# bruniss/multi-task-3d-resencoder-unet

Measured on AMD Instinct MI355X. Metric: train patches/sec (b,c,z,y,x) ResEncM 1x128^3, higher is better.
Workload: dtype bf16; 1 GPU; cfg2: ResEncM (6 stages, feats [32, 64, 128, 256, 512, 512], blocks [1, 3, 4, 6, 6, 6]), 1-in, heads ['sheet'], patch 128x128x128, batch 2/GPU, full train step (fwd+loss+bwd+allreduce+clip+AdamW); global_batch=2, parallelism=dp1

## Files before the change

include/rxunet.h:

```cpp
#ifndef RXUNET_H
#define RXUNET_H

#include <stddef.h>
#include <stdint.h>

#ifdef __cplusplus
extern "C" {
#endif

#define RX_OK 0
#define RX_EINVAL (-1)
#define RX_EUNSUPPORTED (-2)
#define RX_ELAUNCH (-3)
#define RX_EWORKSPACE (-4)

typedef enum { RX_F32 = 0, RX_BF16 = 1, RX_F16 = 2 } rx_dtype;
typedef enum { RX_ACT_NONE = 0, RX_ACT_SIGMOID = 1, RX_ACT_SOFTMAX = 2 } rx_head_act;

typedef struct {
  void* ptr;
  int32_t n, z, y, x, c, ld;
  int64_t cs;
} rx_act;

int rx_abi_version(void);
const char* rx_last_error(void);
int rx_device_arch_ok(void);
const char* rx_last_conv_kernel(void);

int rx_pack_conv_weight(rx_dtype dt, const float* w, int co, int ci, int taps, void* w_fwd, void* w_bwd,
                        void* stream);
int rx_pack_convT_weight(rx_dtype dt, const float* w, int ci, int co, int taps, void* w_fwd, void* w_bwd,
                         void* stream);
int rx_pack_multi(rx_dtype dt, int count, const float* const* w, const int* kind, const int* A, const int* B,
                  const int* taps, void* const* w_fwd, void* const* w_bwd, void* stream);

size_t rx_conv_workspace_hint(void);
int rx_conv3d_fwd(rx_dtype dt, const rx_act* x, const void* w_fwd, const float* bias, const rx_act* y,
                  const int32_t kernel[3], const int32_t stride[3], void* ws, size_t ws_bytes, void* stream);
int rx_conv3d_fwd_stats(rx_dtype dt, const rx_act* x, const void* w_fwd, const float* bias, const rx_act* y,
                        const int32_t kernel[3], const int32_t stride[3], float eps, float* stats, void* ws,
                        size_t ws_bytes, void* stream);
int rx_conv3d_bwd_data(rx_dtype dt, const rx_act* dy, const void* w_bwd, const rx_act* dx,
                       const int32_t kernel[3], const int32_t stride[3], int accumulate, void* ws,
                       size_t ws_bytes, void* stream);
int rx_conv3d_bwd_data_instats(rx_dtype dt, const rx_act* dy, const void* w_bwd, const rx_act* dx,
                               const int32_t kernel[3], const int32_t stride[3], int accumulate, const rx_act* in_y,
                               const float* in_stats, float slope, float* m12, int* fused, void* ws, size_t ws_bytes,
                               void* stream);
size_t rx_conv3d_bwd_weight_workspace(const rx_act* x, const rx_act* dy, const int32_t kernel[3]);
int rx_conv3d_bwd_weight(rx_dtype dt, const rx_act* x, const rx_act* dy, float* dw, const int32_t kernel[3],
                         const int32_t stride[3], void* ws, size_t ws_bytes, void* stream);

int rx_convT3d_fwd(rx_dtype dt, const rx_act* x, const void* w_fwd, const float* bias, const rx_act* y,
                   const int32_t stride[3], void* ws, size_t ws_bytes, void* stream);
int rx_convT3d_bwd_data(rx_dtype dt, const rx_act* dy, const void* w_bwd, const rx_act* dx,
                        const int32_t stride[3], int accumulate, void* ws, size_t ws_bytes, void* stream);
size_t rx_convT3d_bwd_weight_workspace(const rx_act* x, const rx_act* dy, const int32_t stride[3]);
int rx_convT3d_bwd_weight(rx_dtype dt, const rx_act* x, const rx_act* dy, float* dw, const int32_t stride[3],
                          void* ws, size_t ws_bytes, void* stream);

size_t rx_instnorm_stats_workspace(const rx_act* y);
int rx_instnorm_stats(rx_dtype dt, const rx_act* y, float eps, float* stats, void* ws, size_t ws_bytes,
                      void* stream);
int rx_instnorm_stats_mask(float* stats, const float* keep, int count, void* stream);
int rx_instnorm_act_fwd(rx_dtype dt, const rx_act* y, const float* stats, const rx_act* residual,
                        const rx_act* out, float slope, void* stream);
int rx_instnorm_fwd(rx_dtype dt, const rx_act* y, float eps, float* stats, const rx_act* residual,
                    const rx_act* out, float slope, void* ws, size_t ws_bytes, void* stream);
int rx_instnorm_act_bwd(rx_dtype dt, const rx_act* g, const rx_act* y, const float* stats, const rx_act* out,
                        float slope, const rx_act* dy, const rx_act* d_residual, int accumulate_residual,
                        void* ws, size_t ws_bytes, void* stream);

int rx_instnorm_act_bwd_res(rx_dtype dt, const rx_act* g, const rx_act* y, const float* stats, const rx_act* out,
                            float slope, const rx_act* pool_dy, const int32_t pool_stride[3], const rx_act* d_residual,
                            const rx_act* dy, void* ws, size_t ws_bytes, void* stream);

int rx_instnorm_act_bwd_apply(rx_dtype dt, const rx_act* g, const rx_act* y, const float* stats, const rx_act* out,
                              float slope, const float* m12, const rx_act* dy, const rx_act* d_residual,
                              int accumulate_residual, void* stream);

typedef struct {
  const float* w1;
  const float* b1;
  const float* w2;
// ... 144 lines not shown
```

multi-task-3d-resencoder-unet_amd/csrc/rx_wgrad_halo.hip:

```cpp
#include <stdlib.h>

#include <type_traits>

#include "rx_common.h"

struct WgHaloGeom {
  int N, Z, Y, X;
  int R, Cc, ldg, ldx;
  long g_ss, x_ss;
  long x_cs;
  int TZ, TY, TX, lTX, lTY;
  int HY, HX, HV, VT;
  int tz_n, ty_n, tx_n, NT;
  int S, tiles_per_split, panels_c;
  int sz, sy, sx;
  int Zi, Yi, Xi;
  int order;
  int dbg;
};

typedef __attribute__((address_space(3))) s16x4 lds_s16x4_h;

#define RX_WGH_MAX_HV 768
#define RX_WGH_MAX_VT 256
#define RX_WGH_XPIECES ((RX_WGH_MAX_HV * 4 + 255) / 256)
#define RX_WGH_GPIECES (RX_WGH_MAX_VT * 4 / 256)

template <typename T>
__device__ inline u32x4 tr_frag(const T* p0, const T* p1) {
  s16x4 t0 = __builtin_amdgcn_ds_read_tr16_b64_v4i16((lds_s16x4_h*)(p0));
  s16x4 t1 = __builtin_amdgcn_ds_read_tr16_b64_v4i16((lds_s16x4_h*)(p1));
  u32x2 lo = __builtin_bit_cast(u32x2, t0), hi = __builtin_bit_cast(u32x2, t1);
  return u32x4{lo[0], lo[1], hi[0], hi[1]};
}

template <typename T>
__global__ __launch_bounds__(256, 2) void wgrad_halo_kernel(const T* __restrict__ gt, const T* __restrict__ xt, float* __restrict__ slab,
                                                            float* __restrict__ dw, const WgHaloGeom g) {
  extern __shared__ __attribute__((aligned(16))) unsigned char smem[];
  T* sG = reinterpret_cast<T*>(smem);
  T* sX = sG + RX_WGH_MAX_VT * 32;

  const int tid = threadIdx.x, lane = tid & 63;
  const int wave = __builtin_amdgcn_readfirstlane(tid >> 6);
  const int PPn = gridDim.x, lid = rx_xcd_remap(blockIdx.y * PPn + blockIdx.x, PPn * gridDim.y);
  const int split = lid / PPn, pp = lid - split * PPn;
  const int pr = pp / g.panels_c, pc = pp - pr * g.panels_c;
  const int r0 = pr * 32, c0 = pc * 32;
  const long xc0 = g.x_cs ? (long)pc * g.x_cs : (long)c0;
  const int t_begin = split * g.tiles_per_split;
  const int t_end = min(g.NT, t_begin + g.tiles_per_split);

  const int chunk = tid & 3;
  int xh[RX_WGH_XPIECES];
#pragma unroll
  for (int p = 0; p < RX_WGH_XPIECES; ++p) {
    int row = (tid >> 2) + 64 * p;
    if (row < g.HV) {
      int hx = row % g.HX, t = row / g.HX;
      int hy = t % g.HY, hz = t / g.HY;
      xh[p] = (hz << 16) | (hy << 8) | hx;
    } else
      xh[p] = -1;
  }

  const int g16 = lane >> 4, half = g16 & 1, h = g16 >> 1, l15 = lane & 15, q4 = l15 >> 2, p4 = l15 & 3;
  const int coloff = 16 * half + 4 * p4;
  int toff[7];
#pragma unroll
  for (int j = 0; j < 7; ++j) {
    int t = wave + 4 * j;
    int dz = t / 9 - 1, dy = (t / 3) % 3 - 1, dx = t % 3 - 1;
    toff[j] = t < 27 ? ((dz * g.HY + dy) * g.HX + dx) * 32 : 0;
  }

  f32x16 acc[7];
#pragma unroll
  for (int j = 0; j < 7; ++j)
#pragma unroll
// ... 43 lines not shown
      int row = (tid >> 2) + 64 * p;
      if (xh[p] >= 0) *reinterpret_cast<u32x4*>(sX + row * 32 + chunk * 8) = xv[p];
    }
    __syncthreads();
    if (tile + 1 < t_end) load_tile(tile + 1);
    for (int s = 0; s < ksteps; ++s) {
      const int v = 16 * s + 8 * h + q4;
      const int vx = v & (g.TX - 1), vy = (v >> g.lTX) & (g.TY - 1), vz = v >> (g.lTX + g.lTY);
      const int hr = ((vz * g.sz + 1) * g.HY + (vy * g.sy + 1)) * g.HX + vx * g.sx + 1;
      int hr4;
      if (g.TX >= 8)
        hr4 = hr + 4 * g.sx;
      else {
        const int v2 = v + 4;
        const int vy2 = (v2 >> g.lTX) & (g.TY - 1), vz2 = v2 >> (g.lTX + g.lTY);
        hr4 = ((vz2 * g.sz + 1) * g.HY + (vy2 * g.sy + 1)) * g.HX + (v2 & (g.TX - 1)) * g.sx + 1;
      }
      const u32x4 a = tr_frag<T>(sG + v * 32 + coloff, sG + (v + 4) * 32 + coloff);
      const T* b0 = sX + hr * 32 + coloff;
      const T* b1 = sX + hr4 * 32 + coloff;
      u32x4 bf[7];
#pragma unroll
      for (int j = 0; j < 7; ++j)
        if (j < 6 || wave < 3) bf[j] = tr_frag<T>(b0 + toff[j], b1 + toff[j]);
      __builtin_amdgcn_sched_barrier(0);
#pragma unroll
      for (int j = 0; j < 7; ++j)
        if (j < 6 || wave < 3) Mma<T>::run(acc[j], a, bf[j]);
      __builtin_amdgcn_sched_barrier(0);
    }
  }

  const int col = lane & 31, fh = lane >> 5;
  if (g.S == 1) {
    float* sT = reinterpret_cast<float*>(smem);
#pragma unroll
    for (int hb = 0; hb < 2; ++hb) {
      __syncthreads();
#pragma unroll
      for (int j = 0; j < 7; ++j) {
        const int t = wave + 4 * j;
        if (t < 27) {
#pragma unroll
          for (int r = 8 * hb; r < 8 * hb + 8; ++r) {
            const int lr = (r & 3) + 8 * ((r >> 2) & 1) + 4 * fh;
            sT[(lr * 32 + col) * 27 + t] = acc[j][r];
          }
        }
      }
      __syncthreads();
      for (int idx = tid; idx < 16 * 216; idx += 256) {
        const int lr = idx / 216, i = idx - lr * 216;
        *reinterpret_cast<f32x4*>(dw + ((long)(r0 + 16 * hb + lr) * g.Cc + c0) * 27 + 4 * i) = *reinterpret_cast<const f32x4*>(sT + 4 * idx);
      }
    }
    return;
  }
#pragma unroll
  for (int j = 0; j < 7; ++j) {
    const int t = wave + 4 * j;
    if (t < 27) {
      float* out = slab + (((long)split * 27 + t) * g.R + r0) * g.Cc + c0;
#pragma unroll
      for (int r = 0; r < 16; ++r) {
        const int row = (r & 3) + 8 * (r >> 2) + 4 * fh;
        out[(long)row * g.Cc + col] = acc[j][r];
      }
    }
  }
}


typedef __attribute__((address_space(3))) unsigned char lds_byte;

__device__ inline u32x4 tr_frag_at(const lds_byte* p, int off0, int off1) {
  s16x4 t0 = __builtin_amdgcn_ds_read_tr16_b64_v4i16((lds_s16x4_h*)(p + off0));
  s16x4 t1 = __builtin_amdgcn_ds_read_tr16_b64_v4i16((lds_s16x4_h*)(p + off1));
  u32x2 lo = __builtin_bit_cast(u32x2, t0), hi = __builtin_bit_cast(u32x2, t1);
  return u32x4{lo[0], lo[1], hi[0], hi[1]};
}

#define WGH16_HY 6
#define WGH16_HX 18
#define WGH16_HV 648
#define WGH16_XPIECES 11

template <typename T, int W, typename Stage>
__device__ __forceinline__ void wgh16_tile_mma(const lds_byte* gb, const lds_byte* xb, f32x16 (&acc)[7], Stage&& stage) {
  constexpr int NT = W < 3 ? 7 : 6;
  u32x4 fa[2], fb[7];
  auto read_a = [&](int s) { return tr_frag_at(gb, s * 1024, s * 1024 + 256); };
  auto read_b = [&](int s, int j) {
    const int vy = s & 3, vz = s >> 2;
    const int t = W + 4 * j;
    const int dz = t / 9, dy = (t / 3) % 3, dx = t % 3;
    const int off = (((vz + dz) * WGH16_HY + (vy + dy)) * WGH16_HX + dx) * 64;
    return tr_frag_at(xb, off, off + 256);
  };
  fa[0] = read_a(0);
#pragma unroll
  for (int j = 0; j < NT; ++j) fb[j] = read_b(0, j);
#pragma unroll
// ... 283 lines not shown
                        ((long)g.N * g.x_ss + (g.x_cs ? (long)(g.Cc / 32 - 1) * g.x_cs : 0)) * 2 < 0x7fffff00L;
    if (dma_ok && dt == RX_BF16)
      hipLaunchKernelGGL((wgrad_halo16ws_kernel<bf16_t, true>), grid, dim3(512), 2 * lds16, st, (const bf16_t*)dy->ptr, (const bf16_t*)x->ptr, (float*)ws, dw, g);
    else if (dma_ok)
      hipLaunchKernelGGL((wgrad_halo16ws_kernel<f16_t, true>), grid, dim3(512), 2 * lds16, st, (const f16_t*)dy->ptr, (const f16_t*)x->ptr, (float*)ws, dw, g);
    else if (dt == RX_BF16)
      hipLaunchKernelGGL((wgrad_halo16ws_kernel<bf16_t, false>), grid, dim3(512), 2 * lds16, st, (const bf16_t*)dy->ptr, (const bf16_t*)x->ptr, (float*)ws, dw, g);
    else
      hipLaunchKernelGGL((wgrad_halo16ws_kernel<f16_t, false>), grid, dim3(512), 2 * lds16, st, (const f16_t*)dy->ptr, (const f16_t*)x->ptr, (float*)ws, dw, g);
    if (g.S > 1) rx_wgrad_reduce_launch((const float*)ws, g.S, 27, g.R, g.Cc, dw, st);
    hipError_t e16 = hipGetLastError();
    if (e16 != hipSuccess) {
      rx_set_error("wgrad_halo16: %s", hipGetErrorString(e16));
      return RX_ELAUNCH;
    }
    return 1;
  }
  rx_note_kernel("wgrad_halo_kernel");
  if (dt == RX_BF16) {
    (void)hipFuncSetAttribute(reinterpret_cast<const void*>(&wgrad_halo_kernel<bf16_t>), hipFuncAttributeMaxDynamicSharedMemorySize, (int)lds);
    hipLaunchKernelGGL((wgrad_halo_kernel<bf16_t>), grid, dim3(256), lds, st, (const bf16_t*)dy->ptr, (const bf16_t*)x->ptr, (float*)ws, dw, g);
  } else {
    (void)hipFuncSetAttribute(reinterpret_cast<const void*>(&wgrad_halo_kernel<f16_t>), hipFuncAttributeMaxDynamicSharedMemorySize, (int)lds);
    hipLaunchKernelGGL((wgrad_halo_kernel<f16_t>), grid, dim3(256), lds, st, (const f16_t*)dy->ptr, (const f16_t*)x->ptr, (float*)ws, dw, g);
  }
  if (g.S > 1) rx_wgrad_reduce_launch((const float*)ws, g.S, 27, g.R, g.Cc, dw, st);
  hipError_t e = hipGetLastError();
  if (e != hipSuccess) {
    rx_set_error("wgrad_halo: %s", hipGetErrorString(e));
    return RX_ELAUNCH;
  }
  return 1;
}
```

multi-task-3d-resencoder-unet_amd/engine/lib.py:

```python
import ctypes
import os
from ctypes import POINTER, c_char_p, c_double, c_float, c_int, c_int32, c_long, c_size_t, c_void_p

import torch

_HERE = os.path.dirname(os.path.abspath(__file__))
LIB_PATH = os.environ.get("RX_LIBRARY") or os.path.join(os.path.dirname(_HERE), "csrc", "librxunet.so")

RX_F32, RX_BF16, RX_F16 = 0, 1, 2
RX_ACT_NONE, RX_ACT_SIGMOID, RX_ACT_SOFTMAX = 0, 1, 2
DTYPE_CODE = {torch.float32: RX_F32, torch.bfloat16: RX_BF16, torch.float16: RX_F16}
RX_SW_U8, RX_SW_U16, RX_SW_F32 = 0, 1, 2
RX_SW_SCALE, RX_SW_ZSCORE = 0, 1
RX_SW_BLEND_AVERAGE, RX_SW_BLEND_UNIT, RX_SW_BLEND_NONE = 0, 1, 2
RX_SW_CAST_U8, RX_SW_CAST_U16 = 0, 1
RX_AUG_PW_NONE, RX_AUG_PW_AFFINE, RX_AUG_PW_PLANE, RX_AUG_PW_NOISE = 0, 1, 2, 3
RX_AUG_G3_NONE, RX_AUG_G3_FILTER, RX_AUG_G3_DOWNSCALE = 0, 1, 2
RX_AUG_MAX_K, RX_AUG_MAX_BOXES = 21, 4


class RxError(RuntimeError):
    pass


class RxAct(ctypes.Structure):
    _fields_ = [("ptr", c_void_p), ("n", c_int32), ("z", c_int32), ("y", c_int32), ("x", c_int32),
                ("c", c_int32), ("ld", c_int32), ("cs", ctypes.c_int64)]


class RxSeParams(ctypes.Structure):
    _fields_ = [("w1", c_void_p), ("b1", c_void_p), ("w2", c_void_p), ("b2", c_void_p), ("rd", c_int32),
                ("keep_x", c_int32)]


I3 = c_int32 * 3
_P = POINTER(RxAct)
_PSE = POINTER(RxSeParams)

_SIGNATURES = {
    "rx_abi_version": (c_int, []),
    "rx_last_error": (c_char_p, []),
    "rx_device_arch_ok": (c_int, []),
    "rx_last_conv_kernel": (c_char_p, []),
    "rx_pack_conv_weight": (c_int, [c_int, c_void_p, c_int, c_int, c_int, c_void_p, c_void_p, c_void_p]),
    "rx_pack_convT_weight": (c_int, [c_int, c_void_p, c_int, c_int, c_int, c_void_p, c_void_p, c_void_p]),
    "rx_pack_multi": (c_int, [c_int, c_int, c_void_p, c_void_p, c_void_p, c_void_p, c_void_p, c_void_p, c_void_p, c_void_p]),
    "rx_conv_workspace_hint": (c_size_t, []),
    "rx_conv3d_fwd": (c_int, [c_int, _P, c_void_p, c_void_p, _P, I3, I3, c_void_p, c_size_t, c_void_p]),
    "rx_conv3d_fwd_stats": (c_int, [c_int, _P, c_void_p, c_void_p, _P, I3, I3, c_float, c_void_p, c_void_p, c_size_t, c_void_p]),
    "rx_conv3d_bwd_data": (c_int, [c_int, _P, c_void_p, _P, I3, I3, c_int, c_void_p, c_size_t, c_void_p]),
    "rx_conv3d_bwd_data_instats": (c_int, [c_int, _P, c_void_p, _P, I3, I3, c_int, _P, c_void_p, c_float, c_void_p, POINTER(c_int),
                                           c_void_p, c_size_t, c_void_p]),
    "rx_instnorm_act_bwd_apply": (c_int, [c_int, _P, _P, c_void_p, _P, c_float, c_void_p, _P, _P, c_int, c_void_p]),
    "rx_conv3d_bwd_weight_workspace": (c_size_t, [_P, _P, I3]),
    "rx_conv3d_bwd_weight": (c_int, [c_int, _P, _P, c_void_p, I3, I3, c_void_p, c_size_t, c_void_p]),
    "rx_convT3d_fwd": (c_int, [c_int, _P, c_void_p, c_void_p, _P, I3, c_void_p, c_size_t, c_void_p]),
    "rx_convT3d_bwd_data": (c_int, [c_int, _P, c_void_p, _P, I3, c_int, c_void_p, c_size_t, c_void_p]),
    "rx_convT3d_bwd_weight_workspace": (c_size_t, [_P, _P, I3]),
    "rx_convT3d_bwd_weight": (c_int, [c_int, _P, _P, c_void_p, I3, c_void_p, c_size_t, c_void_p]),
    "rx_instnorm_stats_workspace": (c_size_t, [_P]),
    "rx_instnorm_stats": (c_int, [c_int, _P, c_float, c_void_p, c_void_p, c_size_t, c_void_p]),
    "rx_instnorm_act_fwd": (c_int, [c_int, _P, c_void_p, _P, _P, c_float, c_void_p]),
    "rx_instnorm_stats_mask": (c_int, [c_void_p, c_void_p, c_int, c_void_p]),
    "rx_instnorm_fwd": (c_int, [c_int, _P, c_float, c_void_p, _P, _P, c_float, c_void_p, c_size_t, c_void_p]),
    "rx_instnorm_act_bwd": (c_int, [c_int, _P, _P, c_void_p, _P, c_float, _P, _P, c_int, c_void_p, c_size_t,
                                    c_void_p]),
    "rx_instnorm_act_bwd_res": (c_int, [c_int, _P, _P, c_void_p, _P, c_float, _P, I3, _P, _P, c_void_p, c_size_t, c_void_p]),
    "rx_se_workspace": (c_size_t, [_P]),
    "rx_se_gate_fwd": (c_int, [c_int, _P, c_void_p, c_void_p, _PSE, c_void_p, c_void_p, c_void_p, c_void_p, c_void_p, c_size_t,
                               c_void_p]),
    "rx_instnorm_gate_act_fwd": (c_int, [c_int, _P, c_void_p, c_void_p, c_int, _P, _P, c_float, c_void_p]),
    "rx_se_gate_bwd": (c_int, [c_int, _P, _P, c_void_p, _P, c_float, c_void_p, _PSE, c_void_p, c_void_p, c_void_p, c_void_p,
                               c_void_p, c_void_p, c_void_p, c_void_p, c_void_p, c_void_p, c_void_p, c_size_t, c_void_p]),
    "rx_instnorm_gate_act_bwd": (c_int, [c_int, _P, _P, c_void_p, _P, c_float, c_void_p, c_void_p, c_void_p, c_int, _P, _P,
                                         c_int, c_void_p]),
    "rx_avgpool_fwd": (c_int, [c_int, _P, _P, I3, c_void_p]),
    "rx_instnorm_act_pool_fwd": (c_int, [c_int, _P, c_void_p, _P, _P, _P, I3, c_float, c_void_p]),
    "rx_avgpool_bwd": (c_int, [c_int, _P, _P, I3, c_int, c_void_p]),
    "rx_stem_conv_fwd": (c_int, [c_int, c_void_p, c_int, c_int, c_int, c_int, c_int, c_void_p, c_void_p, _P, I3,
                                 c_void_p]),
    "rx_stem_conv_fwd_stats": (c_int, [c_int, c_void_p, c_int, c_int, c_int, c_int, c_int, c_void_p, c_void_p, _P, I3,
                                       c_float, c_void_p, c_void_p, c_size_t, c_void_p]),
    "rx_stem_conv_bwd_weight_workspace": (c_size_t, [c_int, c_int, c_int]),
    "rx_stem_conv_bwd_weight": (c_int, [c_int, c_void_p, c_int, c_int, c_int, c_int, c_int, _P, c_void_p, I3,
                                        c_void_p, c_size_t, c_void_p]),
    "rx_head_fwd": (c_int, [c_int, _P, c_void_p, c_void_p, c_int, c_void_p, c_int, c_void_p]),
    "rx_head_bwd_workspace": (c_size_t, [_P, c_int]),
    "rx_instnorm_act_head_fwd": (c_int, [c_int, _P, c_void_p, _P, c_float, c_void_p, c_void_p, c_int, c_void_p, c_int, c_void_p]),
# ... 100 lines not shown
```

multi-task-3d-resencoder-unet_amd/engine/ops.py:

```python
from ctypes import byref, c_void_p

import numpy as np
import torch

from . import lib as _l
from .lib import I3, RxAct, check, load, stream_ptr

_WS = {}
_PROF = None


def set_profiler(p):
    global _PROF
    _PROF = p


class LaunchProfiler:

    def __init__(self):
        self.pending = []
        self.groups = {}
        self.pending_hbm = []
        self.hbm = {}

# ... 302 lines not shown

    def go():
        check(load().rx_conv3d_bwd_data_instats(_code(dy.dtype), byref(dy.desc()), _ptr(w_bwd), byref(dx.desc()), I3(*kernel),
                                                I3(*stride), int(accumulate), byref(in_y.desc()), _ptr(in_stats), float(slope),
                                                _ptr(m12), byref(fused), *_ws_args(ws), stream_ptr()), "rx_conv3d_bwd_data_instats")
    if _PROF is None:
        go()
    else:
        n = dx.dims[0]
        _PROF.run("dgrad:" + LaunchProfiler.igemm_name(dx.voxels, dx.c), 2.0 * n * dx.voxels * dx.c * dy.c * _taps(kernel), 1, go)
    return bool(fused.value)


def instnorm_act_bwd_apply(g, y, stats, out, dy, m12, slope=0.01, d_residual=None, accumulate_residual=False):
    check(load().rx_instnorm_act_bwd_apply(_code(y.dtype), byref(g.desc()), byref(y.desc()), _ptr(stats),
                                           byref(out.desc()) if out is not None else None, float(slope), _ptr(m12),
                                           byref(dy.desc()),
                                           byref(d_residual.desc()) if d_residual is not None else None,
                                           int(accumulate_residual), stream_ptr()), "rx_instnorm_act_bwd_apply")


def conv3d_bwd_weight(x, dy, dw, kernel, stride, ws=None):
    need = load().rx_conv3d_bwd_weight_workspace(byref(x.desc()), byref(dy.desc()), I3(*kernel))
    ws = workspace(need) if ws is None else ws

    def go():
        check(load().rx_conv3d_bwd_weight(_code(x.dtype), byref(x.desc()), byref(dy.desc()), _ptr(dw), I3(*kernel),
                                          I3(*stride), *_ws_args(ws), stream_ptr()), "rx_conv3d_bwd_weight")
    if _PROF is None:
        return go()
    n = dy.dims[0]
    name = f"wgrad:wgrad_kernel<{64 if dy.c % 64 == 0 else 32},{64 if x.c % 64 == 0 else 32}>"
    _PROF.run(name, 2.0 * n * dy.voxels * dy.c * x.c * _taps(kernel), 1, go)


def convT3d_fwd(x, w_fwd, bias, y, stride, ws=None):
    ws = workspace() if ws is None else ws
    check(load().rx_convT3d_fwd(_code(x.dtype), byref(x.desc()), _ptr(w_fwd), _ptr(bias), byref(y.desc()),
                                I3(*stride), *_ws_args(ws), stream_ptr()), "rx_convT3d_fwd")


def convT3d_bwd_data(dy, w_bwd, dx, stride, accumulate=False, ws=None):
    ws = workspace() if ws is None else ws
    check(load().rx_convT3d_bwd_data(_code(dy.dtype), byref(dy.desc()), _ptr(w_bwd), byref(dx.desc()), I3(*stride),
                                     int(accumulate), *_ws_args(ws), stream_ptr()), "rx_convT3d_bwd_data")


def convT3d_bwd_weight(x, dy, dw, stride, ws=None):
    need = load().rx_convT3d_bwd_weight_workspace(byref(x.desc()), byref(dy.desc()), I3(*stride))
    ws = workspace(need) if ws is None else ws
    check(load().rx_convT3d_bwd_weight(_code(x.dtype), byref(x.desc()), byref(dy.desc()), _ptr(dw), I3(*stride),
                                       *_ws_args(ws), stream_ptr()), "rx_convT3d_bwd_weight")


def instnorm_stats(y, stats, eps=1e-5, ws=None):
    ws = workspace() if ws is None else ws
    check(load().rx_instnorm_stats(_code(y.dtype), byref(y.desc()), eps, _ptr(stats), *_ws_args(ws), stream_ptr()),
          "rx_instnorm_stats")


def instnorm_stats_mask(stats, keep):
    check(load().rx_instnorm_stats_mask(_ptr(stats), _ptr(keep), int(keep.numel()), stream_ptr()), "rx_instnorm_stats_mask")


def instnorm_act_fwd(y, stats, out, slope=0.01, residual=None):
    check(load().rx_instnorm_act_fwd(_code(y.dtype), byref(y.desc()), _ptr(stats),
# ... 309 lines not shown
```

multi-task-3d-resencoder-unet_amd/engine/plan.py:

```python
from dataclasses import dataclass, field
from typing import Callable, Dict, List, Optional

import os

import torch
from torch import nn

from . import lib as _l
from . import ops
from .ops import Act


class UnsupportedConfig(NotImplementedError):
    pass


_SIDE_STREAMS: Dict[str, "torch.cuda.Stream"] = {}


def side_stream(device):
    key = str(device)
    st = _SIDE_STREAMS.get(key)
    if st is None:
        st = _SIDE_STREAMS[key] = torch.cuda.Stream(device=device)
# ... 48 lines not shown
            _l.require_device()
        self.net = net
        self.dtype = dtype
        self.device = device
        self.needs_grad = needs_grad
        self.in_shape = tuple(in_shape)
        self.generation = 0
        self.two_d = net.op_dims == 2
        B, Cin = in_shape[0], in_shape[1]
        spatial = tuple(in_shape[2:])
        if self.two_d:
            spatial = (1,) + spatial
        self.B, self.Cin, self.spatial = B, Cin, spatial

        self.params: List[nn.Parameter] = []
        self._pidx: Dict[int, int] = {}
        self.packs: List[dict] = []
        self.enc_tape: List[Rec] = []
        self.dec_tapes: List[List[Rec]] = []
        self.fwd: List[Callable] = []
        self.bwd: List[Callable] = []
        self.dy_pool: Dict[tuple, Act] = {}
        self._gbase: Dict[int, torch.Tensor] = {}
        self.outputs: Dict[str, torch.Tensor] = {}
        self.bytes_alloc = 0
        self._x = None
        self._dlogits: Dict[str, torch.Tensor] = {}
        self._grads: List[Optional[torch.Tensor]] = []
        self.grad_order: List[int] = []
        self.grad_sync = None
        import os
        self.overlap_wgrad = os.environ.get("RX_OVERLAP_WGRAD", "1") != "0"
        self.dy_ring = 4
        self._side = None
        self._ws2 = None
        self._dy_turn: Dict[tuple, int] = {}
        self._dy_free: Dict[int, int] = {}
        self._dy_ev: Dict[int, int] = {}
        self._ev_fork = None
        self._ev_join = None
        self._pack_groups = None
        self._gates: List[dict] = []
        self._drops: List[dict] = []
        self._shadows: List[dict] = []
        self._shadow_of: Dict[int, dict] = {}
        self._pad_idx: Dict[int, dict] = {}
        self._pad_done: List[int] = []
        self.use_programs = os.environ.get("RX_PROGRAMS", "1") == "1"
        self._pstate: Dict[tuple, dict] = {}
        self._gflat = None
        self._gviews: Dict[int, torch.Tensor] = {}
        self._marks: List[tuple] = []
        self._recording = None
        self._on_side = False
        self._use_gstore = False
        self._gflat_range = (0, 0)
        self._pack_slots: List[int] = []
        self._unstable_params = False
        self._ws_refs: List[object] = []
        self._raw_seen = None
        self.use_graphs = os.environ.get("RX_GRAPHS", "0") == "1"
        self._gstate: Dict[tuple, dict] = {}
        self._x_static = None
        self._dl_static: Dict[str, torch.Tensor] = {}
        self._image_t = None
        self._pack_delay_at = None
# ... 491 lines not shown
                            ops.instnorm_act_fwd(a["y"].act, a["stats"], a["out"].act, a["slope"], res)
                        elif a["drop"] is not None and a["drop"]["active"]:
                            ops.instnorm_stats(a["y"].act, a["stats"], P._eps_now(a))
                            P._mask_dropped(a)
                            ops.instnorm_act_fwd(a["y"].act, a["stats"], a["out"].act, a["slope"], res)
                        else:
                            ops.instnorm_fwd(a["y"].act, a["stats"], a["out"].act, a["slope"], res, a["eps"])
                    f.append(step)
                elif rec.kind == "pool":
                    if not a.get("fused"):
                        f.append(lambda a=a: ops.avgpool_fwd(a["x"].act, a["y"].act, a["stride"]))
                elif rec.kind == "copy":
                    f.append(lambda a=a: ops.avgpool_fwd(a["x"].act, a["y"].act, (1, 1, 1)))
                elif rec.kind == "head":
                    if a.get("fwd_fused"):
                        continue

                    def step(a=a):
                        w2 = a["w"].view(a["k"], -1)
                        ops.head_fwd(a["x"].act, w2, a["b"], a["out"], a["act"] if P._apply_act else _l.RX_ACT_NONE)
                    f.append(step)

    def _dy_for(self, y: AT):
        key = (y.act.dims, y.act.c)
        turn = self._dy_turn.get(key, 0)
        self._dy_turn[key] = (turn + 1) % self.dy_ring
        slot = key + (turn,)
        if slot not in self.dy_pool:
            t = torch.empty((*y.act.dims, y.act.c), dtype=self.dtype, device=self.device)
            self.bytes_alloc += t.numel() * t.element_size()
            self.dy_pool[slot] = Act(t)
        return self.dy_pool[slot]

    def _gen_backward(self):
        P = self
        b = self.bwd
        cat_written = {}

        def mark_cat(cat):
            cat_written[cat.act.key] = True

        def view_written(at):
            return at.written or cat_written.get(at.act.key, False)

        def new_grad(idx):
            sync = P.grad_sync
            ent = P._pad_idx.get(idx)
            if ent is not None:
                if ent["gpad"] is None:
                    ent["gpad"] = torch.empty(tuple(ent["sh"].shape), dtype=torch.float32, device=P.device)
                P._pad_done.append(idx)
                return ent["gpad"]
            if sync is not None:
                g = sync.alloc(idx)
            elif P._use_gstore:
                g = P._gviews[idx]
            else:
                g = torch.empty_like(P.params[idx], memory_format=torch.contiguous_format)
            P._grads[idx] = g
            return g

        skip = set(filter(None, os.environ.get("RX_SKIP", "").split(",")))
        if skip and os.environ.get("RX_ABLATION", "0") != "1":
            raise _l.RxError("RX_SKIP drops launches from the backward pass (timing ablations, wrong gradients): "
                             "set RX_ABLATION=1 as well to confirm, or unset RX_SKIP")

# ... 2 lines not shown
                return
            if P._recording is not None:
                P._marks.append((len(P._recording), idx, P._on_side))
            if P.grad_sync is not None:
                P.grad_sync.ready(idx)

        dy_free = self._dy_free

        def side_run(fn, dy_act):
            if not (P.overlap_wgrad and P._side is not None):
                fn(ops.workspace())
                return
            ops.event_record(P._ev_fork)
            ops.stream_wait(P._ev_fork, P._side)
            key = id(dy_act.t)
            slot = P._dy_ev.get(key)
            if slot is None:
                slot = P._dy_ev[key] = ops.event_new()
            P._on_side = True
            try:
                with torch.cuda.stream(P._side):
                    fn(P._ws2)
                    ops.event_record(slot)
            finally:
                P._on_side = False
            dy_free[key] = slot

        def before_dy_write(dy_act):
            slot = dy_free.pop(id(dy_act.t), None)
            if slot is not None:
                ops.stream_wait(slot)

        order = self.grad_order

        def wrote(at, kind, info=None):
            at._gw = (kind, info)

        for tape in self.dec_tapes + [self.enc_tape]:
            for rec in reversed(tape):
                a = rec.a
                if rec.kind == "head":
                    x = a["x"]
                    assert not view_written(x)
                    gx = self._grad_buf(x)
                    x.written = True
                    hinfo = {"fused": False}
                    wrote(x, "head", hinfo)
                    a["hinfo"] = hinfo

                    def step(a=a, gx=gx, hinfo=hinfo):
                        dl = P._dlogits.get(a["name"])
                        if dl is None:
                            gx.t.zero_()
                            if P.grad_sync is not None:
                                for i in (a["widx"], a["bidx"]):
                                    new_grad(i).zero_()
                                    done(i)
                            return
                        if hinfo.get("dw_fused"):
                            return
                        dw, db = new_grad(a["widx"]), new_grad(a["bidx"])
                        ops.head_bwd(dl, a["x"].act, a["w"].view(a["k"], -1), None if hinfo["fused"] else gx, dw, db)
                        done(a["widx"])
                        done(a["bidx"])
                    order += [a["widx"], a["bidx"]]
                    b.append(step)
                elif rec.kind == "inact":
                    out, y, res = a["out"], a["y"], a["res"]
                    gout = self._grad_buf(out) if out.gact is None else out.gact
                    if not view_written(out):
                        raise RuntimeError(f"plan bug: gradient of {out.name} is consumed before it is produced")
                    dy = self._dy_for(y)
                    y.gact = dy
                    gres, acc = None, False
                    if res is not None and res.needs_grad:
                        gres = self._grad_buf(res)
                        acc = view_written(res)
                        res.written = True
                        wrote(res, "gres")
                    gw = getattr(out, "_gw", (None, None))
                    if (gw[0] == "head" and a["gate"] is None and res is None and self.dtype != torch.float32
                            and out.act.voxels > 512):
                        heads = [r.a for r in tape if r.kind == "head" and r.a["x"] is out]
                        if len(heads) == 1 and heads[0]["k"] <= 4:
                            a["head_src"] = heads[0]
                            gw[1]["fused"] = True
                            if heads[0].get("fwd_fused") and heads[0]["w"] is self.params[heads[0]["widx"]]:
                                a["head_dw_fused"] = True
                                gw[1]["dw_fused"] = True
                    if (gw[0] == "conv" and a["gate"] is None and res is None and self.dtype != torch.float32
                            and out.act.full_buffer and out.act.root is None and out.act.c % 32 == 0 and out.act.voxels > 512
                            and out.act.dims[3] >= 16):
                        a["m12"] = torch.empty((self.B, out.act.c, 2), dtype=torch.float32, device=self.device)
                        a["m12_valid"] = False
                        gw[1]["inact"] = a
                    def gistep(a=a, gout=gout, dy=dy, gres=gres, acc=acc):
                        g = a["gate"]
                        before_dy_write(dy)
                        if g["se"] is None and g.get("scale_now") is None:
                            ops.instnorm_act_bwd(gout, a["y"].act, a["stats"],
                                                 a["out"].act if (a["slope"] != 1.0 and a["res"] is not None) else None, dy,
                                                 a["slope"], gres, acc)
                            return
                        grads = [new_grad(i) for i in g["se"]["idx"]] if g["se"] is not None else [None] * 4
                        ops.se_gate_bwd(gout, a["y"].act, a["stats"], a["out"].act, a["slope"], P._se_args(g), g["pooled"],
# ... 22 lines not shown
                            ops.instnorm_act_bwd_res(gout, a["y"].act, a["stats"], a["out"].act, dy, gres, a["slope"],
                                                     pool_dy=pend["gy"] if pend is not None else None,
                                                     pool_stride=pend["stride"] if pend is not None else (1, 1, 1))
                        b.append(rstep)
                        continue

                    def istep(a=a, gout=gout, dy=dy, gres=gres, acc=acc):
                        before_dy_write(dy)
                        mask_out = a["out"].act if (a["slope"] != 1.0 and a["res"] is not None) else None
                        hs = a.get("head_src")
                        dl = P._dlogits.get(hs["name"]) if hs is not None else None
                        if dl is not None and a.get("head_dw_fused"):
                            dw, db = new_grad(hs["widx"]), new_grad(hs["bidx"])
                            ops.instnorm_act_bwd_head(dl, hs["w"].view(hs["k"], -1), a["y"].act, a["stats"], dy, a["slope"],
                                                      dw=dw.view(hs["k"], -1), db=db)
                            done(hs["widx"])
                            done(hs["bidx"])
                        elif dl is not None:
                            ops.instnorm_act_bwd_head(dl, hs["w"].view(hs["k"], -1), a["y"].act, a["stats"], dy, a["slope"])
                        elif a.get("m12_valid"):
                            a["m12_valid"] = False
                            ops.instnorm_act_bwd_apply(gout, a["y"].act, a["stats"], mask_out, dy, a["m12"], a["slope"], gres, acc)
                        elif "inbwd_reduce" in skip and a["y"].act.voxels > 512:
                            if "m12x" not in a:
                                a["m12x"] = torch.zeros((self.B, a["y"].act.c, 2), dtype=torch.float32, device=self.device)
                            ops.instnorm_act_bwd_apply(gout, a["y"].act, a["stats"], mask_out, dy, a["m12x"], a["slope"], gres, acc)
                        else:
                            ops.instnorm_act_bwd(gout, a["y"].act, a["stats"], mask_out, dy, a["slope"], gres, acc)
                    b.append(istep)
                elif rec.kind in ("conv", "stem"):
                    y = a["y"]
                    dy = y.gact

                    def wstep(a=a, dy=dy, kind=rec.kind):
                        dw = new_grad(a["widx"])
                        db = new_grad(a["bidx"]) if a["bidx"] is not None else None

                        def launches(ws):
                            if "wgrad" in skip and kind != "stem":
                                pass
                            elif kind == "stem":
                                ops.stem_conv_bwd_weight(P._x, dy, dw, a["kernel"], ws)
                            else:
                                ops.conv3d_bwd_weight(a["x"].act, dy, dw, a["kernel"], a["stride"], ws)
                            done(a["widx"])
                            if db is not None:
                                ops.channel_sum(dy, db, ws)
                                done(a["bidx"])
                        side_run(launches, dy)
                    order += [a["widx"]] + ([a["bidx"]] if a["bidx"] is not None else [])
                    b.append(wstep)
                    if rec.kind == "conv" and a["x"].needs_grad:
                        x = a["x"]
                        gx = self._grad_buf(x)
                        acc = view_written(x)
                        x.written = True
                        if x.act.full_buffer:
                            mark_cat(x)
                        bsinfo = {"inact": None}
                        wrote(x, "conv", bsinfo)

                        def dstep(a=a, dy=dy, gx=gx, acc=acc, bsinfo=bsinfo):
                            if "dgrad" in skip:
                                return
                            ia = bsinfo["inact"]
                            if ia is None:
                                ops.conv3d_bwd_data(dy, a["pk"]["w_bwd"], gx, a["kernel"], a["stride"], acc)
                            else:
                                ia["m12_valid"] = ops.conv3d_bwd_data_instats(dy, a["pk"]["w_bwd"], gx, a["kernel"], a["stride"], acc,
                                                                              ia["y"].act, ia["stats"], ia["slope"], ia["m12"])
                        b.append(dstep)
                elif rec.kind == "convT":
                    x, y = a["x"], a["y"]
                    if not view_written(y):
                        raise RuntimeError("plan bug: concat gradient not initialised before the transposed conv")
                    gy = y.act.like(a["cat"].gact.root if a["cat"].gact.root is not None else a["cat"].gact.t)
                    gx = self._grad_buf(x)
                    acc = view_written(x)
                    x.written = True
                    wrote(x, "convT")

                    def step(a=a, gy=gy, gx=gx, acc=acc):
                        dw = new_grad(a["widx"])
# ... 3 lines not shown
                            ops.convT3d_bwd_weight(a["x"].act, gy, dw, a["stride"], ws)
                            done(a["widx"])
                            if db is not None:
                                ops.channel_sum(gy, db, ws)
                                done(a["bidx"])
                        side_run(launches, gy)
                        ops.convT3d_bwd_data(gy, a["pk"]["w_bwd"], gx, a["stride"], acc)
                    order += [a["widx"]] + ([a["bidx"]] if a["bidx"] is not None else [])
                    b.append(step)
                elif rec.kind == "pool":
                    x, y = a["x"], a["y"]
                    if not x.needs_grad:
                        continue
                    gx = self._grad_buf(x)
                    acc = view_written(x)
                    x.written = True
                    wrote(x, "pool")
                    assert y.gact is not None, "plan bug: pooled tensor has no gradient"
                    ti = next(i for i, r in enumerate(tape) if r is rec)
                    prev = tape[ti - 1] if ti > 0 else None
                    if (acc and prev is not None and prev.kind == "inact" and prev.a["out"] is x and prev.a["res"] is not None
                            and prev.a["gate"] is None and x.act.voxels > 512):
                        x._pool_pending = dict(gy=y.gact, gx=gx, stride=a["stride"])
                        continue
                    b.append(lambda a=a, gy=y.gact, gx=gx, acc=acc: ops.avgpool_bwd(gy, gx, a["stride"], acc))
                elif rec.kind == "copy":
                    x, y = a["x"], a["y"]
                    gy = y.act.like(a["cat"].gact.root if a["cat"].gact.root is not None else a["cat"].gact.t)
                    gx = self._grad_buf(x)
                    acc = view_written(x)
                    x.written = True
                    wrote(x, "copy")
                    b.append(lambda gy=gy, gx=gx, acc=acc: ops.avgpool_bwd(gy, gx, (1, 1, 1), acc))

    def _grad_buf(self, at: AT):
        if at.gact is not None:
            return at.gact
        base = at.act.root if at.act.root is not None else at.act.t
        if at.act.key not in self._gbase:
            t = torch.empty_like(base)
            self.bytes_alloc += t.numel() * t.element_size()
            self._gbase[at.act.key] = t
        at.gact = at.act.like(self._gbase[at.act.key])
        return at.gact

    def _ensure_side(self):
        if self.device.type == "cuda" and self.overlap_wgrad and self._side is None:
            self._side = side_stream(self.device)
            self._ws2 = torch.empty(ops.workspace().numel(), dtype=torch.uint8, device=self.device)
        if self._ev_fork is None and self.device.type == "cuda":
            self._ev_fork, self._ev_join = ops.event_new(), ops.event_new()

    def _await_pack(self, ent):
        if ent.get("deferred") and self._pack_deferred is not None:
            self._issue_deferred_packs()
        slot = ent.get("event")
        if slot is not None:
            ops.stream_wait(slot)
            for e in ent["group"]:
                e["event"] = None

    def _packs_stale(self, force=False):
        epoch = getattr(self.net, "_weights_epoch", 0)
        return [e for e in self.packs
                if force or e.get("epoch") != epoch
                or not (e["version"] == e["param"]._version and e.get("ptr") == e["param"].data_ptr())]
# ... 335 lines not shown
                    sync.ready(idx)
            else:
                sync.ready(idx)
        prog.run(streams, pos, -1)

    def run_backward(self, dlogits: Dict[str, Optional[torch.Tensor]]):
        graphs = self._graphs_on()
        programs = (not graphs) and self._programs_on() and all(dlogits.get(k) is not None for k in self.outputs)
        self._dlogits = {}
        for k, g in dlogits.items():
            if g is None:
                continue
            g = g.detach()
            if g.dtype != torch.float32 or not g.is_contiguous():
                g = g.float().contiguous()
            if graphs or programs:
                buf = self._dl_static.get(k)
                if buf is None or buf.shape != g.shape:
                    buf = self._dl_static[k] = torch.empty_like(g)
                buf.copy_(g)
                g = buf
            self._dlogits[k] = g.unsqueeze(2) if self.two_d else g
        self._ensure_side()
        self.net._weights_epoch = getattr(self.net, "_weights_epoch", 0) + 1
        self._grads = [None] * len(self.params)
        if programs:
            sync = self.grad_sync
            self._use_gstore = sync is None
            if sync is None:
                self._grad_store()
            else:
                sync.persistent = True
                sync.begin(self)
            key = ("b", tuple(sorted(self._dlogits)), id(sync) if sync is not None else 0, self.overlap_wgrad)
            st, replayed = self._programmed(key, self._backward_body,
                                            segments=self._replay_backward_segments if sync is not None else None)
            if replayed:
                self._pad_done = [idx for idx in set(self.grad_order) if idx in self._pad_idx]
            if replayed and sync is None:
                for idx in set(self.grad_order):
                    self._grads[idx] = self._gviews[idx]
            grads = self._backward_finish()
            return [t.detach() if t is not None else None for t in grads]
        self._use_gstore = False
        if self.grad_sync is not None:
            self.grad_sync.persistent = False
            self.grad_sync.begin(self)
        if not graphs:
            self._backward_body()
            return self._backward_finish()
        key = ("b", tuple(sorted(self._dlogits)))
        st = self._gstate.get(key)
        if st is not None and st.get("graph") is not None:
            owned = st["owned"]
            for p in self.params:
                gr = p.grad
                if gr is not None and gr.data_ptr() in owned:
                    p.grad = gr.clone()

        def body():
            self._backward_body()
            return self._backward_finish()
        st = self._graphed(key, body)
        grads = st["result"]
        if st["eager"]:
            return grads
        if "owned" not in st:
            st["owned"] = {t.data_ptr() for t in grads if t is not None}
        return [t.detach() if t is not None else None for t in grads]
```

Measured before the change: 117.4 patches/s.

## Batch deep-stage 3x3x3 weight-gradient convs into one grouped kernel launch

Adds a grouped weight-gradient kernel that handles several small, deep-stage 3x3x3 stride-1 convolutions (at most 2048 voxels) in a single launch. A table of entries is indexed by binary search over block offsets. The planner gives each eligible conv its own dy buffer so the gradient stays live until a deferred flush, then emits one grouped launch plus bias sums on the side stream. This targets launch overhead and the low occupancy of many tiny wgrad kernels, at the cost of extra dy memory, delayed gradient availability for allreduce ordering, and no split-K for these layers.

Result: slower. 114.4 patches/s (-2.5%).

```diff
diff --git a/include/rxunet.h b/include/rxunet.h
--- a/include/rxunet.h
+++ b/include/rxunet.h
@@ -51,6 +51,10 @@
 size_t rx_conv3d_bwd_weight_workspace(const rx_act* x, const rx_act* dy, const int32_t kernel[3]);
 int rx_conv3d_bwd_weight(rx_dtype dt, const rx_act* x, const rx_act* dy, float* dw, const int32_t kernel[3],
                          const int32_t stride[3], void* ws, size_t ws_bytes, void* stream);
+int rx_wgrad_group_eligible(rx_dtype dt, const rx_act* x, const rx_act* dy, const int32_t kernel[3],
+                            const int32_t stride[3]);
+int rx_conv3d_bwd_weight_group(rx_dtype dt, int count, const rx_act* x, const rx_act* dy, float* const* dw,
+                               void* stream);
 
 int rx_convT3d_fwd(rx_dtype dt, const rx_act* x, const void* w_fwd, const float* bias, const rx_act* y,
                    const int32_t stride[3], void* ws, size_t ws_bytes, void* stream);
diff --git a/multi-task-3d-resencoder-unet_amd/csrc/rx_wgrad_halo.hip b/multi-task-3d-resencoder-unet_amd/csrc/rx_wgrad_halo.hip
--- a/multi-task-3d-resencoder-unet_amd/csrc/rx_wgrad_halo.hip
+++ b/multi-task-3d-resencoder-unet_amd/csrc/rx_wgrad_halo.hip
@@ -34,17 +34,15 @@
   return u32x4{lo[0], lo[1], hi[0], hi[1]};
 }
 
-template <typename T>
-__global__ __launch_bounds__(256, 2) void wgrad_halo_kernel(const T* __restrict__ gt, const T* __restrict__ xt, float* __restrict__ slab,
-                                                            float* __restrict__ dw, const WgHaloGeom g) {
+template <typename T, bool SINGLE>
+__device__ __forceinline__ void wgh_panel_pair(const T* __restrict__ gt, const T* __restrict__ xt, float* __restrict__ slab,
+                                               float* __restrict__ dw, const WgHaloGeom& g, const int pp, const int split) {
   extern __shared__ __attribute__((aligned(16))) unsigned char smem[];
   T* sG = reinterpret_cast<T*>(smem);
   T* sX = sG + RX_WGH_MAX_VT * 32;
 
   const int tid = threadIdx.x, lane = tid & 63;
   const int wave = __builtin_amdgcn_readfirstlane(tid >> 6);
-  const int PPn = gridDim.x, lid = rx_xcd_remap(blockIdx.y * PPn + blockIdx.x, PPn * gridDim.y);
-  const int split = lid / PPn, pp = lid - split * PPn;
   const int pr = pp / g.panels_c, pc = pp - pr * g.panels_c;
   const int r0 = pr * 32, c0 = pc * 32;
   const long xc0 = g.x_cs ? (long)pc * g.x_cs : (long)c0;
@@ -154,7 +152,7 @@
   }
 
   const int col = lane & 31, fh = lane >> 5;
-  if (g.S == 1) {
+  if (SINGLE || g.S == 1) {
     float* sT = reinterpret_cast<float*>(smem);
 #pragma unroll
     for (int hb = 0; hb < 2; ++hb) {
@@ -190,6 +188,39 @@
       }
     }
   }
+}
+
+template <typename T>
+__global__ __launch_bounds__(256, 2) void wgrad_halo_kernel(const T* __restrict__ gt, const T* __restrict__ xt, float* __restrict__ slab,
+                                                            float* __restrict__ dw, const WgHaloGeom g) {
+  const int PPn = gridDim.x, lid = rx_xcd_remap(blockIdx.y * PPn + blockIdx.x, PPn * gridDim.y);
+  const int split = lid / PPn, pp = lid - split * PPn;
+  wgh_panel_pair<T, false>(gt, xt, slab, dw, g, pp, split);
+}
+
+#define RX_WGG_MAX 16
+struct WgGroupEntry {
+  const void* dy;
+  const void* x;
+  float* dw;
+  WgHaloGeom g;
+};
+struct WgGroupTab {
+  WgGroupEntry e[RX_WGG_MAX];
+  int start[RX_WGG_MAX + 1];
+  int count;
+};
+
+template <typename T>
+__global__ __launch_bounds__(256, 2) void wgrad_halo_group_kernel(const WgGroupTab tab) {
+  const int lid = rx_xcd_remap(blockIdx.x, gridDim.x);
+  int lo = 0, hi = tab.count;
+  while (hi - lo > 1) {
+    const int mid = (lo + hi) >> 1;
+    if (tab.start[mid] <= lid) lo = mid; else hi = mid;
+  }
+  const WgGroupEntry& e = tab.e[lo];
+  wgh_panel_pair<T, true>((const T*)e.dy, (const T*)e.x, nullptr, e.dw, e.g, lid - tab.start[lo], 0);
 }
 
 
@@ -539,3 +570,68 @@
   }
   return 1;
 }
+
+static int wgg_plan(rx_dtype dt, const rx_act* x, const rx_act* dy, const int32_t kernel[3], const int32_t stride[3], WgHaloGeom* g) {
+  if (dt != RX_BF16 && dt != RX_F16) return 0;
+  if (!rx_act_ok(x) || !rx_act_ok(dy) || !kernel || !stride) return 0;
+  for (int i = 0; i < 3; ++i)
+    if (kernel[i] != 3 || stride[i] != 1) return 0;
+  if (dy->n != x->n || dy->z != x->z || dy->y != x->y || dy->x != x->x) return 0;
+  if (x->c % 32 || dy->c % 32 || x->ld % 8 || dy->ld % 8 || ((uintptr_t)x->ptr & 15) || ((uintptr_t)dy->ptr & 15)) return 0;
+  if ((long)dy->n * rx_act_voxels(dy) > 2048) return 0;
+  if (!wgh_plan(x, dy, stride, g, (size_t)-1)) return 0;
+  if (g->TZ == 4 && g->TY == 4 && g->TX == 16) return 0;
+  g->S = 1, g->tiles_per_split = g->NT;
+  g->order = 1;
+  return 1;
+}
+
+extern "C" int rx_wgrad_group_eligible(rx_dtype dt, const rx_act* x, const rx_act* dy, const int32_t kernel[3], const int32_t stride[3]) {
+  WgHaloGeom g;
+  return wgg_plan(dt, x, dy, kernel, stride, &g);
+}
+
+extern "C" int rx_conv3d_bwd_weight_group(rx_dtype dt, int count, const rx_act* x, const rx_act* dy, float* const* dw, void* stream) {
+  if (count < 1 || !x || !dy || !dw) RX_FAIL(RX_EINVAL, "rx_conv3d_bwd_weight_group: bad arguments");
+  RxRecScope rx_scope__;
+  if (rx_scope__.rec) {
+    std::vector<rx_act> x_(x, x + count), dy_(dy, dy + count);
+    std::vector<float*> dw_(dw, dw + count);
+    rx_rec_push(RxCmdFn([=](void* s) { return rx_conv3d_bwd_weight_group(dt, count, x_.data(), dy_.data(), dw_.data(), s); }), stream, __func__);
+  }
+  static const int32_t k3[3] = {3, 3, 3}, s1[3] = {1, 1, 1};
+  hipStream_t st = (hipStream_t)stream;
+  const size_t lds = (size_t)(RX_WGH_MAX_VT + RX_WGH_MAX_HV) * 64;
+  for (int i = 0; i < count; ++i) {
+    WgHaloGeom g;
+    if (!wgg_plan(dt, &x[i], &dy[i], k3, s1, &g))
+      RX_FAIL(RX_EUNSUPPORTED, "rx_conv3d_bwd_weight_group: entry %d is not eligible (see rx_wgrad_group_eligible)", i);
+    if (!dw[i] || ((uintptr_t)dw[i] & 15)) RX_FAIL(RX_EINVAL, "rx_conv3d_bwd_weight_group: dw[%d] is null or not 16-byte aligned", i);
+  }
+  rx_note_kernel("wgrad_halo_group_kernel");
+  for (int i0 = 0; i0 < count; i0 += RX_WGG_MAX) {
+    WgGroupTab t;
+    memset(&t, 0, sizeof(t));
+    const int k = count - i0 < RX_WGG_MAX ? count - i0 : RX_WGG_MAX;
+    long blocks = 0;
+    for (int j = 0; j < k; ++j) {
+      const int i = i0 + j;
+      WgGroupEntry& e = t.e[j];
+      (void)wgg_plan(dt, &x[i], &dy[i], k3, s1, &e.g);
+      e.dy = dy[i].ptr, e.x = x[i].ptr, e.dw = dw[i];
+      t.start[j] = (int)blocks;
+      blocks += (long)(e.g.R / 32) * e.g.panels_c;
+    }
+    for (int q = k; q <= RX_WGG_MAX; ++q) t.start[q] = (int)blocks;
+    t.count = k;
+    if (dt == RX_BF16) {
+      (void)hipFuncSetAttribute(reinterpret_cast<const void*>(&wgrad_halo_group_kernel<bf16_t>), hipFuncAttributeMaxDynamicSharedMemorySize, (int)lds);
+      hipLaunchKernelGGL((wgrad_halo_group_kernel<bf16_t>), dim3((unsigned)blocks), dim3(256), lds, st, t);
+    } else {
+      (void)hipFuncSetAttribute(reinterpret_cast<const void*>(&wgrad_halo_group_kernel<f16_t>), hipFuncAttributeMaxDynamicSharedMemorySize, (int)lds);
+      hipLaunchKernelGGL((wgrad_halo_group_kernel<f16_t>), dim3((unsigned)blocks), dim3(256), lds, st, t);
+    }
+  }
+  RX_CHECK_LAUNCH("rx_conv3d_bwd_weight_group");
+  return RX_OK;
+}
diff --git a/multi-task-3d-resencoder-unet_amd/engine/lib.py b/multi-task-3d-resencoder-unet_amd/engine/lib.py
--- a/multi-task-3d-resencoder-unet_amd/engine/lib.py
+++ b/multi-task-3d-resencoder-unet_amd/engine/lib.py
@@ -54,6 +54,8 @@
     "rx_instnorm_act_bwd_apply": (c_int, [c_int, _P, _P, c_void_p, _P, c_float, c_void_p, _P, _P, c_int, c_void_p]),
     "rx_conv3d_bwd_weight_workspace": (c_size_t, [_P, _P, I3]),
     "rx_conv3d_bwd_weight": (c_int, [c_int, _P, _P, c_void_p, I3, I3, c_void_p, c_size_t, c_void_p]),
+    "rx_wgrad_group_eligible": (c_int, [c_int, _P, _P, I3, I3]),
+    "rx_conv3d_bwd_weight_group": (c_int, [c_int, c_int, _P, _P, c_void_p, c_void_p]),
     "rx_convT3d_fwd": (c_int, [c_int, _P, c_void_p, c_void_p, _P, I3, c_void_p, c_size_t, c_void_p]),
     "rx_convT3d_bwd_data": (c_int, [c_int, _P, c_void_p, _P, I3, c_int, c_void_p, c_size_t, c_void_p]),
     "rx_convT3d_bwd_weight_workspace": (c_size_t, [_P, _P, I3]),
diff --git a/multi-task-3d-resencoder-unet_amd/engine/ops.py b/multi-task-3d-resencoder-unet_amd/engine/ops.py
--- a/multi-task-3d-resencoder-unet_amd/engine/ops.py
+++ b/multi-task-3d-resencoder-unet_amd/engine/ops.py
@@ -358,6 +358,31 @@
     n = dy.dims[0]
     name = f"wgrad:wgrad_kernel<{64 if dy.c % 64 == 0 else 32},{64 if x.c % 64 == 0 else 32}>"
     _PROF.run(name, 2.0 * n * dy.voxels * dy.c * x.c * _taps(kernel), 1, go)
+
+
+WGRAD_GROUP_PER_LAUNCH = 16
+
+
+def wgrad_group_eligible(x, dy, kernel, stride):
+    return bool(load().rx_wgrad_group_eligible(_code(x.dtype), byref(x.desc()), byref(dy.desc()), I3(*kernel), I3(*stride)))
+
+
+def conv3d_bwd_weight_group(items):
+    n = len(items)
+    if n == 0:
+        return
+    xs = (_l.RxAct * n)(*[x.desc() for x, _, _ in items])
+    dys = (_l.RxAct * n)(*[dy.desc() for _, dy, _ in items])
+    dws = (c_void_p * n)(*[dw.data_ptr() for _, _, dw in items])
+
+    def go():
+        check(load().rx_conv3d_bwd_weight_group(_code(items[0][0].dtype), n, xs, dys, dws, stream_ptr()),
+              "rx_conv3d_bwd_weight_group")
+    if _PROF is None:
+        return go()
+    flops = sum(2.0 * dy.dims[0] * dy.voxels * dy.c * x.c * 27 for x, dy, _ in items)
+    launches = (n + WGRAD_GROUP_PER_LAUNCH - 1) // WGRAD_GROUP_PER_LAUNCH
+    _PROF.run("wgrad:wgrad_halo_group_kernel", flops, launches, go)
 
 
 def convT3d_fwd(x, w_fwd, bias, y, stride, ws=None):
diff --git a/multi-task-3d-resencoder-unet_amd/engine/plan.py b/multi-task-3d-resencoder-unet_amd/engine/plan.py
--- a/multi-task-3d-resencoder-unet_amd/engine/plan.py
+++ b/multi-task-3d-resencoder-unet_amd/engine/plan.py
@@ -104,6 +104,8 @@
         import os
         self.overlap_wgrad = os.environ.get("RX_OVERLAP_WGRAD", "1") != "0"
         self.dy_ring = 4
+        self.group_deep_wgrad = True
+        self.group_wgrad_on_side = True
         self._side = None
         self._ws2 = None
         self._dy_turn: Dict[tuple, int] = {}
@@ -661,6 +663,19 @@
             self.dy_pool[slot] = Act(t)
         return self.dy_pool[slot]
 
+    def _dy_own(self, y: AT, tape):
+        if self.device.type != "cuda" or self.dtype == torch.float32:
+            return None
+        rec = next((r for r in tape if r.kind == "conv" and r.a["y"] is y), None)
+        if rec is None or y.act.dims[0] * y.act.voxels > 2048:
+            return None
+        dy = Act(torch.empty((*y.act.dims, y.act.c), dtype=self.dtype, device=self.device))
+        if not ops.wgrad_group_eligible(rec.a["x"].act, dy, rec.a["kernel"], rec.a["stride"]):
+            return None
+        self.bytes_alloc += dy.t.numel() * dy.t.element_size()
+        y._wgroup = True
+        return dy
+
     def _gen_backward(self):
         P = self
         b = self.bwd
@@ -729,6 +744,39 @@
                 ops.stream_wait(slot)
 
         order = self.grad_order
+
+        pending = []
+
+        def flush_group():
+            if not pending:
+                return
+            members = list(pending)
+            pending.clear()
+            for m in members:
+                order.append(m["a"]["widx"])
+            for m in members:
+                if m["a"]["bidx"] is not None:
+                    order.append(m["a"]["bidx"])
+
+            def gstep(members=members):
+                if not P.group_deep_wgrad:
+                    return
+                items = [(m["a"]["x"].act, m["dy"], new_grad(m["a"]["widx"])) for m in members]
+                dbs = [(m, new_grad(m["a"]["bidx"])) for m in members if m["a"]["bidx"] is not None]
+
+                def launches(ws):
+                    if "wgrad" not in skip:
+                        ops.conv3d_bwd_weight_group(items)
+                    for m in members:
+                        done(m["a"]["widx"])
+                    for m, db in dbs:
+                        ops.channel_sum(m["dy"], db, ws)
+                        done(m["a"]["bidx"])
+                if P.group_wgrad_on_side:
+                    side_run(launches, members[-1]["dy"])
+                else:
+                    launches(ops.workspace())
+            b.append(gstep)
 
         def wrote(at, kind, info=None):
             at._gw = (kind, info)
@@ -767,7 +815,7 @@
                     gout = self._grad_buf(out) if out.gact is None else out.gact
                     if not view_written(out):
                         raise RuntimeError(f"plan bug: gradient of {out.name} is consumed before it is produced")
-                    dy = self._dy_for(y)
+                    dy = self._dy_own(y, tape) or self._dy_for(y)
                     y.gact = dy
                     gres, acc = None, False
                     if res is not None and res.needs_grad:
@@ -856,7 +904,15 @@
                     y = a["y"]
                     dy = y.gact
 
-                    def wstep(a=a, dy=dy, kind=rec.kind):
+                    grouped = rec.kind == "conv" and getattr(y, "_wgroup", False)
+                    if grouped:
+                        pending.append(dict(a=a, dy=dy))
+                    elif dy.dims[0] * dy.voxels > 2048:
+                        flush_group()
+
+                    def wstep(a=a, dy=dy, kind=rec.kind, grouped=grouped):
+                        if grouped and P.group_deep_wgrad:
+                            return
                         dw = new_grad(a["widx"])
                         db = new_grad(a["bidx"]) if a["bidx"] is not None else None
 
@@ -872,7 +928,8 @@
                                 ops.channel_sum(dy, db, ws)
                                 done(a["bidx"])
                         side_run(launches, dy)
-                    order += [a["widx"]] + ([a["bidx"]] if a["bidx"] is not None else [])
+                    if not grouped:
+                        order += [a["widx"]] + ([a["bidx"]] if a["bidx"] is not None else [])
                     b.append(wstep)
                     if rec.kind == "conv" and a["x"].needs_grad:
                         x = a["x"]
@@ -942,6 +999,7 @@
                     x.written = True
                     wrote(x, "copy")
                     b.append(lambda gy=gy, gx=gx, acc=acc: ops.avgpool_bwd(gy, gx, (1, 1, 1), acc))
+            flush_group()
 
     def _grad_buf(self, at: AT):
         if at.gact is not None:
@@ -1343,7 +1401,8 @@
             else:
                 sync.persistent = True
                 sync.begin(self)
-            key = ("b", tuple(sorted(self._dlogits)), id(sync) if sync is not None else 0, self.overlap_wgrad)
+            key = ("b", tuple(sorted(self._dlogits)), id(sync) if sync is not None else 0, self.overlap_wgrad,
+                   self.group_deep_wgrad, self.group_wgrad_on_side)
             st, replayed = self._programmed(key, self._backward_body,
                                             segments=self._replay_backward_segments if sync is not None else None)
             if replayed:
@@ -1360,7 +1419,7 @@
         if not graphs:
             self._backward_body()
             return self._backward_finish()
-        key = ("b", tuple(sorted(self._dlogits)))
+        key = ("b", tuple(sorted(self._dlogits)), self.group_deep_wgrad, self.group_wgrad_on_side)
         st = self._gstate.get(key)
         if st is not None and st.get("graph") is not None:
             owned = st["owned"]
```
